# impromptuRong/hd_yolo

Measured on AMD Instinct MI355X. Metric: tiles/sec (640x640) fwd+bwd, higher is better.
Workload: dtype bf16; 1 GPU; metayolo yolov5s 8-class nuclei, 640x640 RGB tiles, batch 64/GPU, train step = fwd + DetLoss + bwd + all-reduce + SGD(nesterov); global_batch=64, parallelism=dp1, world_size=1, backend=none, hw_queues=4

## Files before the change

hd_yolo_amd/build.py:

```python
import os
import subprocess
import sys
from concurrent.futures import ThreadPoolExecutor

HERE = os.path.dirname(os.path.abspath(__file__))
CSRC = os.path.join(HERE, 'csrc')
OUT = os.path.join(CSRC, 'build')
LIB = os.path.join(OUT, 'libhdyolo_hip.so')
SOURCES = ['api.hip', 'conv_dispatch.hip', 'conv_igemm.hip', 'conv3x3.hip', 'conv3x3_c128.hip', 'conv3x3s2.hip', 'conv_deep.hip', 'conv_stem.hip', 'conv_wgrad.hip', 'conv_wgrad3x3.hip', 'conv_wgrad_deep.hip', 'conv_dgrad_s2.hip', 'conv1x1_bwd.hip', 'bn_act.hip', 'pool.hip', 'detect.hip', 'loss.hip', 'roi.hip', 'seg.hip', 'optim.hip', 'exec.hip']
FLAGS = ['--offload-arch=gfx950', '-O3', '-fPIC', '-std=c++17', '-ffp-contract=off', '-Wall', '-Wno-unused-function',
         '-I' + CSRC, '-I' + os.path.join(os.path.dirname(HERE), 'include')]


def _newer(a, bs):
    return os.path.exists(a) and all(os.path.getmtime(a) >= os.path.getmtime(b) for b in bs)


def build(force=False, verbose=True):
    os.makedirs(OUT, exist_ok=True)
    headers = [os.path.join(CSRC, h) for h in os.listdir(CSRC) if h.endswith('.h')]
    headers.append(os.path.join(os.path.dirname(HERE), 'include', 'hdyolo.h'))
    hipcc = os.environ.get('HIPCC', '/opt/rocm/bin/hipcc')

    def compile_one(src):
        s = os.path.join(CSRC, src)
        o = os.path.join(OUT, src.replace('.hip', '.o'))
        if not force and _newer(o, [s] + headers):
            return o
        cmd = [hipcc] + FLAGS + ['-c', s, '-o', o]
        if verbose:
            print(' '.join(cmd), flush=True)
        subprocess.check_call(cmd)
        return o

    with ThreadPoolExecutor(max_workers=min(6, os.cpu_count() or 1)) as ex:
        objs = list(ex.map(compile_one, SOURCES))
    if force or not _newer(LIB, objs):
        cmd = [hipcc, '--offload-arch=gfx950', '-shared', '-fPIC', '-o', LIB] + objs
        if verbose:
            print(' '.join(cmd), flush=True)
        subprocess.check_call(cmd)
    return LIB


if __name__ == '__main__':
    print(build(force='--force' in sys.argv))
```

hd_yolo_amd/csrc/api.hip:

```cpp
#include <stdarg.h>
#include <stdio.h>
#include <stdlib.h>
#include <string.h>

#include <atomic>

#include "common.h"
#include "hdyolo_internal.h"
#include "hdyolo.h"

int hdy_wgrad_reduce_launch(const float* partial, int splits, size_t slab_stride, int K, int Q, int mode, int C, int R, int S, float* grad,
                            int accumulate, hipStream_t st);
int hdy_pack_weight_launch(const hdy_pack_desc& d, hipStream_t st);
int hdy_pack_batch_launch(const hdy_pack_desc* table, int n, int total_blocks, hipStream_t st);

static thread_local char g_err[512] = "";

void hdy_set_error(const char* fmt, ...) {
    va_list ap;
    va_start(ap, fmt);
    vsnprintf(g_err, sizeof(g_err), fmt, ap);
    va_end(ap);
}

namespace {
struct OptDef { const char* name; int def; bool flag; };
const OptDef g_opt_def[HDY_OPT_COUNT] = {
    {"HDY_NO_CLASS_WALK", 0, true}, {"HDY_NO_CONV3X3", 0, true}, {"HDY_C3_GRID", 0, false}, {"HDY_NO_CONV3X3S2", 0, false},
    {"HDY_NO_DGRAD_S2", 0, false}, {"HDY_TILE_INTERLEAVE", 1, false}, {"HDY_NO_BIG_TILES", 0, true}, {"HDY_NO_STEM_KERNEL", 0, true},
    {"HDY_WGRAD_BLOCKS", 512, false}, {"HDY_NO_STEM_WGRAD", 0, true}, {"HDY_NO_WGRAD3X3", 0, true}, 
    {"HDY_LOSS_GRID", 2048, false}, {"HDY_NO_DEEP", 0, true}, {"HDY_NO_WGRAD_S2", 0, true}, {"HDY_NO_WGRAD_DEEP", 0, true}, {"HDY_DEEP_BN", 0, false}, {"HDY_DEEP_DEBUG", 0, false}, {"HDY_DEEP_ALL", 1, false}, {"HDY_DEEP_MIN_TILES", 160, false}, {"HDY_DEEP_WALK", 2, false}, {"HDY_NO_BN_REDUCE4", 0, true},
    {"HDY_WGRAD_TILE", 0, false}, {"HDY_SPPF_NO_KEYS", 0, true}, {"HDY_WGRAD_DEEP_KMIN", 192, false}, {"HDY_NO_CONV3X3_C128", 0, true}, {"HDY_NO_F1X1_96", 0, true},
};
std::atomic<int> g_opt[HDY_OPT_COUNT];
std::once_flag g_opt_once;
void opt_init() {
    std::call_once(g_opt_once, [] {
        for (int i = 0; i < HDY_OPT_COUNT; ++i) {
            const char* v = getenv(g_opt_def[i].name);
            g_opt[i].store(v ? (g_opt_def[i].flag ? 1 : atoi(v)) : g_opt_def[i].def, std::memory_order_relaxed);
        }
    });
}
int opt_index(const char* name) {
    for (int i = 0; name && i < HDY_OPT_COUNT; ++i)
        if (!strcmp(name, g_opt_def[i].name)) return i;
    return -1;
}
thread_local char g_disp_last[64] = "";
std::mutex g_disp_mu;
char g_disp_log[32768] = "";
size_t g_disp_len = 0;
thread_local char g_disp_copy[32768] = "";
}

int hdy_opt(int id) {
    opt_init();
    return g_opt[id].load(std::memory_order_relaxed);
}

void hdy_note_dispatch(const char* what) {
    snprintf(g_disp_last, sizeof(g_disp_last), "%s", what);
    const size_t n = strlen(g_disp_last);
    std::lock_guard<std::mutex> lock(g_disp_mu);
    if (g_disp_len + n + 2 < sizeof(g_disp_log)) {
        memcpy(g_disp_log + g_disp_len, g_disp_last, n);
        g_disp_log[g_disp_len + n] = ';';
        g_disp_log[g_disp_len + n + 1] = 0;
        g_disp_len += n + 1;
    }
}

namespace {

enum { KIND_FWD = 0, KIND_DGRAD = 1, KIND_STEM = 2 };

inline int velems(int dtype) { return dtype == HDY_BF16 ? 8 : 4; }
inline int bke(int dtype) { return 8 * velems(dtype); }
inline size_t esize(int dtype) { return dtype == HDY_BF16 ? 2 : 4; }

struct Axis { int taps, d0, rmax; };
inline Axis class_axis(int R, int pad, int a) {
    Axis ax = {0, 0, -1};
    for (int r = R - 1; r >= 0; --r)
        if (((a + pad - r) & 1) == 0) {
            if (ax.rmax < 0) { ax.rmax = r; ax.d0 = (a + pad - r) / 2; }
            ++ax.taps;
        }
    return ax;
}

inline bool dgrad_class_walk(int H, int W, int R, int S, int pad) {
    if (H % 2 || W % 2 || hdy_opt(HDY_OPT_NO_CLASS_WALK)) return false;
    for (int a = 0; a < 2; ++a)
        if (!class_axis(R, pad, a).taps || !class_axis(S, pad, a).taps) return false;
    return true;
}

inline size_t block_elems(int rows, int kd, int dtype) {
    const int bn = hdy_conv_bn_tile(rows);
    return (size_t)round_up(rows, bn) * round_up(kd, bke(dtype));
}

}

extern "C" {

const char* hdy_last_error(void) { return g_err; }

const char* hdy_last_dispatch(void) { return g_disp_last; }

const char* hdy_dispatch_log(void) {
    std::lock_guard<std::mutex> lock(g_disp_mu);
    memcpy(g_disp_copy, g_disp_log, g_disp_len + 1);
    return g_disp_copy;
}

void hdy_dispatch_log_reset(void) {
    std::lock_guard<std::mutex> lock(g_disp_mu);
    g_disp_log[0] = 0;
    g_disp_len = 0;
    g_disp_last[0] = 0;
}

int hdy_set_option(const char* name, int value) {
    const int i = opt_index(name);
    HDY_ARG(i >= 0, "set_option: unknown option %s", name ? name : "(null)");
    opt_init();
    return g_opt[i].exchange(value, std::memory_order_relaxed);
}

int hdy_get_option(const char* name) {
    const int i = opt_index(name);
    HDY_ARG(i >= 0, "get_option: unknown option %s", name ? name : "(null)");
    return hdy_opt(i);
}

int hdy_version(void) { return HDY_ABI_VERSION; }

int hdy_fastdiv_magic(unsigned d, unsigned* magic, int* shift) {
    HDY_ARG(d > 0 && magic && shift, "fastdiv_magic: d must be positive");
    hdy_magic(d, magic, shift);
    return HDY_OK;
}

int hdy_conv_out_dim(int in, int k, int stride, int pad) { return conv_out_dim(in, k, stride, pad); }

int hdy_conv_mtiles(long long M) { return (int)((M + 127) / 128); }

size_t hdy_conv_pack_elems(int K, int C, int R, int S, int stride, int pad, int kind, int dtype) {
    if (kind == KIND_FWD) return block_elems(K, R * S * C, dtype);
    if (kind == KIND_STEM) return block_elems(K, R * S * 4, dtype);
    if (stride == 1) return block_elems(C, R * S * K, dtype);
    size_t n = 0;
    for (int a = 0; a < 2; ++a)
        for (int b = 0; b < 2; ++b) {
            const Axis ah = class_axis(R, pad, a), aw = class_axis(S, pad, b);
            if (ah.taps && aw.taps) n += block_elems(C, ah.taps * aw.taps * K, dtype);
        }
    return n;
}

static hdy_pack_desc make_desc(const float* w_a, int K_a, const float* w_b, int K_b, void* out, int Kl, int C, int R, int S, int transpose,
                               int TH, int TW, int rbase, int rstep, int sbase, int sstep, int stem, int rows_total, int Kdp, int dtype,
                               int first_block) {
    hdy_pack_desc d = {};
    d.w_a = w_a; d.w_b = w_b; d.out = out; d.K_a = K_a; d.K_b = K_b; d.Kl = Kl; d.C = C; d.R = R; d.S = S; d.transpose = transpose;
    d.TH = TH; d.TW = TW; d.rbase = rbase; d.rstep = rstep; d.sbase = sbase; d.sstep = sstep; d.stem = stem; d.rows_total = rows_total;
    d.Kdp = Kdp; d.dtype = dtype; d.first_block = first_block;
    d.nblocks = cdiv((long long)rows_total * Kdp, 2048);
    return d;
}

int hdy_conv_pack_describe(const float* w_a, int K_a, const float* w_b, int K_b, int K, int C, int R, int S, int stride, int pad, int kind,
                           int dtype, void* out, hdy_pack_desc* descs, int first_block) {
    HDY_ARG(w_a && out && descs && K_a > 0 && K_b >= 0 && K >= K_a + K_b && C > 0 && R > 0 && S > 0, "conv_pack: bad args");
    HDY_ARG((K_b == 0) == (w_b == nullptr), "conv_pack: w_b / K_b mismatch");
    HDY_ARG(stride == 1 || stride == 2, "conv_pack: stride %d unsupported", stride);
    HDY_ARG(dtype == HDY_BF16 || dtype == HDY_F32, "conv_pack: unknown dtype %d", dtype);
    HDY_ARG(((long long)K + 256) * ((long long)R * S * ((long long)C + 256) + 64) < (1LL << 31), "conv_pack: weight too large for 32-bit packing indices");
    if (kind == KIND_FWD || kind == KIND_STEM) {
        const int stem = kind == KIND_STEM;
        HDY_ARG(!stem || (C == 3 && K_b == 0), "conv_pack: stem expects C == 3 and a single weight");
        const int kd = stem ? R * S * 4 : R * S * C;
        const int Kdp = round_up(kd, bke(dtype));
        const int rows_total = round_up(K, hdy_conv_bn_tile(K));
        descs[0] = make_desc(w_a, K_a, w_b, K_b, out, K, C, R, S, 0, R, stem ? 1 : S, 0, 1, 0, 1, stem, rows_total, Kdp, dtype, first_block);
        return 1;
    }
    HDY_ARG(kind == KIND_DGRAD, "conv_pack: unknown kind %d", kind);
    const int rows_total = round_up(C, hdy_conv_bn_tile(C));
    if (stride == 1) {
        const int Kdp = round_up(R * S * K, bke(dtype));
        descs[0] = make_desc(w_a, K_a, w_b, K_b, out, K, C, R, S, 1, R, S, R - 1, -1, S - 1, -1, 0, rows_total, Kdp, dtype, first_block);
        return 1;
    }
    size_t off = 0;
    int n = 0;
    for (int a = 0; a < 2; ++a)
        for (int b = 0; b < 2; ++b) {
            const Axis ah = class_axis(R, pad, a), aw = class_axis(S, pad, b);
            if (!ah.taps || !aw.taps) continue;
            const int Kdp = round_up(ah.taps * aw.taps * K, bke(dtype));
            descs[n] = make_desc(w_a, K_a, w_b, K_b, (char*)out + off * esize(dtype), K, C, R, S, 1, ah.taps, aw.taps, ah.rmax, -2, aw.rmax,
                                 -2, 0, rows_total, Kdp, dtype, first_block);
            first_block += descs[n].nblocks;
            off += (size_t)rows_total * Kdp;
            ++n;
        }
    return n;
}

int hdy_conv_pack(const float* w_a, int K_a, const float* w_b, int K_b, int K, int C, int R, int S, int stride, int pad, int kind,
                  int dtype, void* out, void* stream) {
    hdy_pack_desc d[4];
    const int n = hdy_conv_pack_describe(w_a, K_a, w_b, K_b, K, C, R, S, stride, pad, kind, dtype, out, d, 0);
    if (n < 0) return n;
    for (int i = 0; i < n; ++i) {
        const int rc = hdy_pack_weight_launch(d[i], (hipStream_t)stream);
        if (rc) return rc;
    }
    return HDY_OK;
}

int hdy_conv_pack_run(const hdy_pack_desc* descs_device, int ndesc, int total_blocks, void* stream) {
    HDY_ARG(descs_device && ndesc > 0 && total_blocks > 0, "conv_pack_run: bad args");
    return hdy_pack_batch_launch(descs_device, ndesc, total_blocks, (hipStream_t)stream);
}

int hdy_conv_fwd(const void* x, int ldx, const void* w_packed, const float* scale, const float* shift, const void* res, int ldr, void* y,
                 int ldy, float* stats, int stat_slabs, int N, int H, int W, int C, int K, int R, int S, int stride, int pad, int act, int accumulate,
                 int dtype, int out_f32, int stem, void* stream) {
    HDY_ARG(!stats || stat_slabs > 0, "conv_fwd: stats given with stat_slabs = %d", stat_slabs);
    HDY_ARG(stride >= 1 && R >= 1 && S >= 1 && pad >= 0, "conv_fwd: bad window");
    HDY_ARG(dtype == HDY_BF16 || dtype == HDY_F32, "conv_fwd: unknown dtype %d", dtype);
    ConvArgs a = {};
    a.x = x; a.w = w_packed; a.y = y; a.scale = scale; a.shift = shift; a.stats = stats; a.stat_cap = stat_slabs; a.res = res; a.ldr = ldr;
    HDY_ARG(!res || ldr >= K, "conv_fwd: residual pitch %d < K", ldr);
    a.N = N;
    a.Ho = hdy_conv_out_dim(H, R, stride, pad);
    a.Wo = hdy_conv_out_dim(W, S, stride, pad);
    HDY_ARG(a.Ho > 0 && a.Wo > 0, "conv_fwd: empty output");
    a.K = K; a.ldy = ldy;
    a.Hout = a.Ho; a.Wout = a.Wo; a.oh_mul = a.ow_mul = 1; a.oh_off = a.ow_off = 0; a.dense_out = 1;
    a.act = act; a.accumulate = accumulate;
    if (stem) {
        HDY_ARG(C == 3 && R == 6 && S == 6 && stride == 2 && pad == 2 && ldx == 4, "conv_fwd: stem expects C=3 k=6 s=2 p=2 on a 4-channel padded image");
        a.Hin = H + 2 * pad; a.Win = W + 2 * pad; a.C = 24; a.ldx = 4; a.span_pixels = 1;
        a.ih_mul = 2; a.iw_mul = 2; a.dh0 = 0; a.dw0 = 0; a.TH = 6; a.TW = 1;
        a.Kdp = round_up(6 * 24, bke(dtype));
        return hdy_conv_launch(a, dtype, out_f32, (hipStream_t)stream);
    }
    a.Hin = H; a.Win = W; a.C = C; a.ldx = ldx;
    a.ih_mul = stride; a.iw_mul = stride; a.dh0 = -pad; a.dw0 = -pad; a.TH = R; a.TW = S;
    a.Kdp = round_up(R * S * C, bke(dtype));
    return hdy_conv_launch(a, dtype, out_f32, (hipStream_t)stream);
}

static int dgrad_impl(const void* dy, int lddy, const void* w_packed_dgrad, void* dx, int lddx, int N, int H, int W, int C, int K, int R,
                      int S, int stride, int pad, int accumulate, int dtype, const hdy_stat_req* stats, int nstat, void* stream);

int hdy_conv_dgrad(const void* dy, int lddy, const void* w_packed_dgrad, void* dx, int lddx, int N, int H, int W, int C, int K, int R,
                   int S, int stride, int pad, int accumulate, int dtype, void* stream) {
    return dgrad_impl(dy, lddy, w_packed_dgrad, dx, lddx, N, H, W, C, K, R, S, stride, pad, accumulate, dtype, nullptr, 0, stream);
}

int hdy_conv_dgrad_stats(const void* dy, int lddy, const void* w_packed_dgrad, void* dx, int lddx, int N, int H, int W, int C, int K, int R,
                         int S, int stride, int pad, int accumulate, int dtype, const hdy_stat_req* stats, int nstat, void* stream) {
    HDY_ARG(nstat >= 0 && nstat <= 2 && (nstat == 0 || stats), "conv_dgrad_stats: bad request count");
    HDY_ARG(nstat == 0 || hdy_conv_dgrad_stat_slabs(N, H, W, C, K, R, S, stride, pad, dtype) > 0, "conv_dgrad_stats: this shape cannot serve statistics");
    return dgrad_impl(dy, lddy, w_packed_dgrad, dx, lddx, N, H, W, C, K, R, S, stride, pad, accumulate, dtype, stats, nstat, stream);
}

int hdy_conv_dgrad_stat_slabs(int N, int H, int W, int C, int K, int R, int S, int stride, int pad, int dtype) {
    if (dtype != HDY_BF16 || C % 8 || hdy_conv_bn_tile(C) > 64 || (stride != 1 && stride != 2)) return 0;
    if (stride == 2 && !dgrad_class_walk(H, W, R, S, pad)) return 0;
    ConvShape s = {};
    s.N = N; s.Ho = H / stride; s.Wo = W / stride; s.C = K; s.K = C; s.R = R; s.S = S; s.stride = 1; s.pad = -1; s.dtype = dtype;
    s.dense = stride == 1; s.ncls = stride == 2 ? 4 : 1;
    ConvPlan p;
    hdy_conv_igemm_plan(s, &p);
    return p.grid;
}

static int dgrad_impl(const void* dy, int lddy, const void* w_packed_dgrad, void* dx, int lddx, int N, int H, int W, int C, int K, int R,
                      int S, int stride, int pad, int accumulate, int dtype, const hdy_stat_req* stats, int nstat, void* stream) {
    HDY_ARG(stride == 1 || stride == 2, "conv_dgrad: stride %d unsupported", stride);
    HDY_ARG(dtype == HDY_BF16 || dtype == HDY_F32, "conv_dgrad: unknown dtype %d", dtype);
    const int Ho = hdy_conv_out_dim(H, R, stride, pad), Wo = hdy_conv_out_dim(W, S, stride, pad);
    HDY_ARG(Ho > 0 && Wo > 0, "conv_dgrad: empty dy");
    ConvArgs a = {};
    a.x = dy; a.y = dx; a.N = N; a.Hin = Ho; a.Win = Wo; a.C = K; a.ldx = lddy;
    a.K = C; a.ldy = lddx; a.Hout = H; a.Wout = W;
    a.ih_mul = a.iw_mul = 1; a.accumulate = accumulate;
    a.nstat = nstat;
    for (int r = 0; r < nstat; ++r)
        a.stat[r] = StatReq{stats[r].y, stats[r].ldy, stats[r].scale, stats[r].shift, stats[r].slabs, stats[r].c0, stats[r].c1, stats[r].act, stats[r].nslabs};
    if (stride == 1) {
        a.w = w_packed_dgrad;
        a.Ho = H; a.Wo = W; a.oh_mul = a.ow_mul = 1; a.dense_out = 1;
        a.dh0 = pad - (R - 1); a.dw0 = pad - (S - 1); a.TH = R; a.TW = S;
        a.Kdp = round_up(R * S * K, bke(dtype));
        return hdy_conv_launch(a, dtype, 0, (hipStream_t)stream);
    }
    const int rows_total = round_up(C, hdy_conv_bn_tile(C));
    size_t off = 0;
    if (dgrad_class_walk(H, W, R, S, pad)) {
        ConvArgs c = a;
        c.ncls = 4;
        c.Ho = H / 2; c.Wo = W / 2;
        c.oh_mul = c.ow_mul = 2; c.dense_out = 0;
        for (int ca = 0; ca < 2; ++ca)
            for (int cb = 0; cb < 2; ++cb) {
                const Axis ah = class_axis(R, pad, ca), aw = class_axis(S, pad, cb);
                const int i = ca * 2 + cb;
                const int Kdp = round_up(ah.taps * aw.taps * K, bke(dtype));
                c.c_dh[i] = ah.d0; c.c_dw[i] = aw.d0; c.c_TH[i] = ah.taps; c.c_TW[i] = aw.taps;
                c.c_nkb[i] = Kdp / bke(dtype); c.c_oh[i] = ca; c.c_ow[i] = cb; c.c_w[i] = (long long)off;
                off += (size_t)rows_total * Kdp;
            }
        c.w = w_packed_dgrad;
        c.dh0 = c.c_dh[0]; c.dw0 = c.c_dw[0]; c.TH = c.c_TH[0]; c.TW = c.c_TW[0]; c.oh_off = c.ow_off = 0;
        c.Kdp = c.c_nkb[0] * bke(dtype);
        int rc2 = HDY_OK;
        if (hdy_dgrad3x3s2_try(c, dtype, (hipStream_t)stream, &rc2)) return rc2;
        return hdy_conv_launch(c, dtype, 0, (hipStream_t)stream);
    }
    for (int ca = 0; ca < 2; ++ca)
        for (int cb = 0; cb < 2; ++cb) {
            const Axis ah = class_axis(R, pad, ca), aw = class_axis(S, pad, cb);
            ConvArgs c = a;
            c.Ho = (H - ca + 1) / 2; c.Wo = (W - cb + 1) / 2;
            c.oh_mul = c.ow_mul = 2; c.oh_off = ca; c.ow_off = cb; c.dense_out = 0;
            if (!ah.taps || !aw.taps) {
                HDY_ARG(false, "conv_dgrad: kernel %dx%d pad %d leaves a parity class without taps (unsupported)", R, S, pad);
            }
            if (c.Ho <= 0 || c.Wo <= 0) continue;
            c.dh0 = ah.d0; c.dw0 = aw.d0; c.TH = ah.taps; c.TW = aw.taps;
            c.Kdp = round_up(ah.taps * aw.taps * K, bke(dtype));
            c.w = (const char*)w_packed_dgrad + off * esize(dtype);
            off += (size_t)rows_total * c.Kdp;
            const int rc = hdy_conv_launch(c, dtype, 0, (hipStream_t)stream);
            if (rc) return rc;
        }
    return HDY_OK;
}

size_t hdy_conv_wgrad_workspace_bytes(int N, int H, int W, int C, int K, int R, int S, int stride, int pad, int dtype, int stem) {
    const int Ho = hdy_conv_out_dim(H, R, stride, pad), Wo = hdy_conv_out_dim(W, S, stride, pad);
    const int Q = stem ? R * S * 4 : R * S * C;
    int splits = 1, pps = 64;
    hdy_wgrad_plan(K, Q, (long long)N * Ho * Wo, dtype, &splits, &pps);
    if (stem) {
        const int g = hdy_wgrad_stem_grid(N, Ho, Wo, K, dtype);
        if (g > splits) splits = g;
    }
    size_t bytes = (size_t)splits * K * Q * sizeof(float);
    if (!stem && R == 3 && S == 3 && pad == 1) {
        const size_t b3 = hdy_wgrad3x3_workspace_bytes(N, Ho, Wo, C, K, stride, dtype);
        if (b3 > bytes) bytes = b3;
    }
    if (!stem) {
        const size_t bd = hdy_wgrad_deep_workspace_bytes(N, H, W, Ho, Wo, C, K, R, S, stride, dtype);
        if (bd > bytes) bytes = bd;
    }
    return bytes;
}

int hdy_conv_wgrad(const void* x, int ldx, const void* dy, int lddy, int N, int H, int W, int C, int K, int R, int S, int stride, int pad,
                   float* grad_a, int K_a, float* grad_b, int K_b, int accumulate, void* workspace, size_t ws_bytes, int dtype, int stem,
                   void* stream) {
    HDY_ARG(grad_a && K_a > 0 && K_a + K_b <= K && K_b >= 0 && (K_b == 0) == (grad_b == nullptr), "conv_wgrad: bad gradient split");
    HDY_ARG(dtype == HDY_BF16 || dtype == HDY_F32, "conv_wgrad: unknown dtype %d", dtype);
    HDY_ARG(workspace && ws_bytes >= hdy_conv_wgrad_workspace_bytes(N, H, W, C, K, R, S, stride, pad, dtype, stem), "conv_wgrad: workspace too small");
    WgradArgs a = {};
    a.x = x; a.dy = dy; a.partial = (float*)workspace;
    a.N = N; a.K = K; a.lddy = lddy;
    a.Ho = hdy_conv_out_dim(H, R, stride, pad);
    a.Wo = hdy_conv_out_dim(W, S, stride, pad);
    HDY_ARG(a.Ho > 0 && a.Wo > 0, "conv_wgrad: empty dy");
    if (stem) {
        HDY_ARG(C == 3 && R == 6 && S == 6 && stride == 2 && pad == 2 && ldx == 4, "conv_wgrad: stem expects C=3 k=6 s=2 p=2 on a 4-channel padded image");
        a.Hin = H + 2 * pad; a.Win = W + 2 * pad; a.C = 24; a.ldx = 4; a.span_pixels = 1;
        a.ih_mul = a.iw_mul = 2; a.dh0 = a.dw0 = 0; a.TH = 6; a.TW = 1;
    } else {
        a.Hin = H; a.Win = W; a.C = C; a.ldx = ldx;
        a.ih_mul = a.iw_mul = stride; a.dh0 = a.dw0 = -pad; a.TH = R; a.TW = S;
    }
    const int Q = a.TH * a.TW * a.C;
    const int stem_grid = stem ? hdy_wgrad_stem_grid(N, a.Ho, a.Wo, K, dtype) : 0;
    int rc;
    if (!stem && R == 3 && S == 3 && pad == 1 &&
        hdy_wgrad3x3_try(x, ldx, dy, lddy, N, H, W, a.Ho, a.Wo, C, K, stride, a.partial, dtype, (hipStream_t)stream, &a.splits, &rc)) {
    } else if (!stem && hdy_wgrad_deep_try(x, ldx, dy, lddy, N, H, W, a.Ho, a.Wo, C, K, R, S, stride, pad, a.partial, dtype, (hipStream_t)stream, &a.splits, &rc)) {
    } else if (stem_grid > 0) {
        a.splits = stem_grid;
        rc = hdy_wgrad_stem_launch(a, stem_grid, (hipStream_t)stream);
    } else {
        hdy_wgrad_plan(K, Q, (long long)N * a.Ho * a.Wo, dtype, &a.splits, &a.pix_per_split);
        rc = hdy_wgrad_launch(a, dtype, (hipStream_t)stream);
    }
    if (rc) return rc;
    const int mode = stem ? 1 : 0;
    rc = hdy_wgrad_reduce_launch(a.partial, a.splits, (size_t)K * Q, K_a, Q, mode, C, R, S, grad_a, accumulate, (hipStream_t)stream);
    if (rc) return rc;
    if (K_b) {
        rc = hdy_wgrad_reduce_launch(a.partial + (size_t)K_a * Q, a.splits, (size_t)K * Q, K_b, Q, mode, C, R, S, grad_b, accumulate,
                                     (hipStream_t)stream);
    }
    return rc;
}

int hdy_conv_wgrad_stem_fused_ok(int N, int H, int W, int K) {
    if (K != 16 && K != 32 && K != 64) return 0;
    const int Ho = hdy_conv_out_dim(H, 6, 2, 2), Wo = hdy_conv_out_dim(W, 6, 2, 2);
    return hdy_wgrad_stem_grid(N, Ho, Wo, K, HDY_BF16) > 0 ? 1 : 0;
}

int hdy_conv_wgrad_stem_fused(const void* x, const void* dz, int lddz, const void* y, int ldy, const float* scale, const float* shift, const float* mean,
                              const float* invstd, const float* c1, const float* c2, int N, int H, int W, int K, float* grad_a, int K_a, float* grad_b,
                              int K_b, int accumulate, void* workspace, size_t ws_bytes, void* stream) {
    HDY_ARG(x && dz && y && grad_a && K_a > 0 && K_a + K_b <= K && K_b >= 0 && (K_b == 0) == (grad_b == nullptr), "conv_wgrad_stem_fused: bad arguments");
    HDY_ARG(hdy_conv_wgrad_stem_fused_ok(N, H, W, K), "conv_wgrad_stem_fused: shape not served (K in {16, 32, 64}, output a multiple of 16 x 32)");
    HDY_ARG(workspace && ws_bytes >= hdy_conv_wgrad_workspace_bytes(N, H, W, 3, K, 6, 6, 2, 2, HDY_BF16, 1), "conv_wgrad_stem_fused: workspace too small");
    WgradArgs a = {};
    a.x = x; a.dy = dz; a.lddy = lddz; a.partial = (float*)workspace;
    a.y = y; a.ldy = ldy; a.bn_scale = scale; a.bn_shift = shift; a.bn_mean = mean; a.bn_invstd = invstd; a.bn_c1 = c1; a.bn_c2 = c2;
    a.N = N; a.K = K;
    a.Ho = hdy_conv_out_dim(H, 6, 2, 2);
    a.Wo = hdy_conv_out_dim(W, 6, 2, 2);
    a.Hin = H + 4; a.Win = W + 4; a.C = 24; a.ldx = 4; a.span_pixels = 1;
    a.ih_mul = a.iw_mul = 2; a.dh0 = a.dw0 = 0; a.TH = 6; a.TW = 1;
    const int Q = a.TH * a.TW * a.C;
    a.splits = hdy_wgrad_stem_grid(N, a.Ho, a.Wo, K, HDY_BF16);
    int rc = hdy_wgrad_stem_launch(a, a.splits, (hipStream_t)stream);
    if (rc) return rc;
    rc = hdy_wgrad_reduce_launch(a.partial, a.splits, (size_t)K * Q, K_a, Q, 1, 3, 6, 6, grad_a, accumulate, (hipStream_t)stream);
    if (rc) return rc;
    if (K_b) rc = hdy_wgrad_reduce_launch(a.partial + (size_t)K_a * Q, a.splits, (size_t)K * Q, K_b, Q, 1, 3, 6, 6, grad_b, accumulate, (hipStream_t)stream);
    return rc;
}

}
```

hd_yolo_amd/csrc/common.h:

```cpp
#pragma once
#include <hip/hip_runtime.h>
#include <stdint.h>
#include <stddef.h>

#include <mutex>

#define HDY_OK 0
#define HDY_EINVAL (-1)
#define HDY_EUNSUPPORTED (-2)

enum { HDY_F32 = 0, HDY_BF16 = 1 };

void hdy_set_error(const char* fmt, ...);

enum HdyOption {
    HDY_OPT_NO_CLASS_WALK,
    HDY_OPT_NO_CONV3X3,
    HDY_OPT_C3_GRID,
    HDY_OPT_NO_CONV3X3S2,
    HDY_OPT_NO_DGRAD_S2,
    HDY_OPT_TILE_INTERLEAVE,
    HDY_OPT_NO_BIG_TILES,
    HDY_OPT_NO_STEM_KERNEL,
    HDY_OPT_WGRAD_BLOCKS,
    HDY_OPT_NO_STEM_WGRAD,
    HDY_OPT_NO_WGRAD3X3,
    HDY_OPT_LOSS_GRID,
    HDY_OPT_NO_DEEP,
    HDY_OPT_NO_WGRAD_S2,
    HDY_OPT_NO_WGRAD_DEEP,
    HDY_OPT_DEEP_BN,
    HDY_OPT_DEEP_DEBUG,
    HDY_OPT_DEEP_ALL,
    HDY_OPT_DEEP_MIN_TILES,
    HDY_OPT_DEEP_WALK,
    HDY_OPT_NO_BN_REDUCE4,
    HDY_OPT_WGRAD_TILE,
    HDY_OPT_SPPF_NO_KEYS,
    HDY_OPT_WGRAD_DEEP_KMIN,
    HDY_OPT_NO_CONV3X3_C128,
    HDY_OPT_NO_F1X1_96,
    HDY_OPT_COUNT
};
int hdy_opt(int id);

void hdy_note_dispatch(const char* what);

#define HDY_ARG(cond, ...)                 \
    do {                                   \
        if (!(cond)) {                     \
            hdy_set_error(__VA_ARGS__);    \
            return HDY_EINVAL;             \
        }                                  \
    } while (0)

#define HDY_LAUNCH_CHECK(what)                                                       \
    do {                                                                             \
        hipError_t e__ = hipGetLastError();                                          \
        if (e__ != hipSuccess) {                                                     \
            hdy_set_error("%s: launch failed: %s", what, hipGetErrorString(e__));    \
            return (int)e__;                                                         \
        }                                                                            \
    } while (0)

typedef __bf16 bf16_t;
typedef int i32x4 __attribute__((ext_vector_type(4)));
typedef float f32x4 __attribute__((ext_vector_type(4)));
typedef __bf16 bf16x8 __attribute__((ext_vector_type(8)));
typedef __bf16 bf16x4 __attribute__((ext_vector_type(4)));

#if defined(__HIPCC__)
__device__ __forceinline__ float row_sum16(float v) {
#ifdef HDY_ROW_SUM_SHFL
    for (int m = 1; m < 16; m <<= 1) v += __shfl_xor(v, m);
    return v;
#endif
    v += __builtin_bit_cast(float, __builtin_amdgcn_update_dpp(0, __builtin_bit_cast(int, v), 0x128, 0xF, 0xF, true));
    v += __builtin_bit_cast(float, __builtin_amdgcn_update_dpp(0, __builtin_bit_cast(int, v), 0x124, 0xF, 0xF, true));
    v += __builtin_bit_cast(float, __builtin_amdgcn_update_dpp(0, __builtin_bit_cast(int, v), 0x122, 0xF, 0xF, true));
    v += __builtin_bit_cast(float, __builtin_amdgcn_update_dpp(0, __builtin_bit_cast(int, v), 0x121, 0xF, 0xF, true));
    return v;
}
#endif

struct PerDeviceOnce {
    std::once_flag flag[16];
    template <typename F> void run(F&& fn) {
        int dev = 0;
        (void)hipGetDevice(&dev);
        std::call_once(flag[dev & 15], fn);
    }
};

static inline int cdiv(long long a, long long b) { return (int)((a + b - 1) / b); }
static inline int round_up(int a, int b) { return (a + b - 1) / b * b; }

#ifdef __HIPCC__
union V16 {
    i32x4 i;
    f32x4 f;
    bf16x8 h;
};

__device__ __forceinline__ float silu_f(float u) { return u / (1.0f + __expf(-u)); }
__device__ __forceinline__ float sigmoid_f(float u) { return 1.0f / (1.0f + __expf(-u)); }

template <typename T> __device__ __forceinline__ float to_f32(T v);
template <> __device__ __forceinline__ float to_f32<float>(float v) { return v; }
template <> __device__ __forceinline__ float to_f32<bf16_t>(bf16_t v) { return (float)v; }
template <typename T> __device__ __forceinline__ T from_f32(float v);
template <> __device__ __forceinline__ float from_f32<float>(float v) { return v; }
template <> __device__ __forceinline__ bf16_t from_f32<bf16_t>(float v) { return (bf16_t)v; }

__device__ __forceinline__ int xcd_remap(int id, int n) {
    const int q = n >> 3, r = n & 7, x = id & 7, s = id >> 3;
    return (x < r ? x * (q + 1) : r * (q + 1) + (x - r) * q) + s;
}
__device__ __forceinline__ unsigned fdiv(unsigned n, unsigned mg, int sh) { return __umulhi(n << 1, mg) >> sh; }

__device__ __forceinline__ void glds16(const void* g, unsigned char* lds_wave_base) {
    __builtin_amdgcn_global_load_lds((const void __attribute__((address_space(1)))*)g,
                                     (void __attribute__((address_space(3)))*)lds_wave_base, 16, 0, 0);
}

__device__ __forceinline__ void lds_dma16(__amdgpu_buffer_rsrc_t r, unsigned voff, unsigned soff, unsigned char* lds_wave_base) {
    __builtin_amdgcn_raw_ptr_buffer_load_lds(r, (void __attribute__((address_space(3)))*)lds_wave_base, 16, (int)voff, (int)soff, 0, 0);
}

__device__ __forceinline__ void lds_dma16(__amdgpu_buffer_rsrc_t r, unsigned voff, unsigned soff, unsigned lds_byte) {
    __builtin_amdgcn_raw_ptr_buffer_load_lds(r, (void __attribute__((address_space(3)))*)(uintptr_t)lds_byte, 16, (int)voff, (int)soff, 0, 0);
}

__device__ __forceinline__ int fsw(int row) { return ((row >> 1) & 1) | (((row >> 3) & 1) << 1); }
__device__ __forceinline__ int fsw3(int row) { return (row & 6) ^ (((row >> 3) & 1) * 5); }

__device__ __forceinline__ float fast_sigmoid(float u) { return __builtin_amdgcn_rcpf(1.0f + __expf(-u)); }
__device__ __forceinline__ float dsilu_f(float u) {
    const float s = fast_sigmoid(u);
    return s * (1.0f + u * (1.0f - s));
}

template <typename T> __device__ __forceinline__ void unpack(const i32x4& v, float* f);
template <> __device__ __forceinline__ void unpack<float>(const i32x4& v, float* f) {
    V16 u; u.i = v;
#pragma unroll
    for (int i = 0; i < 4; ++i) f[i] = u.f[i];
}
template <> __device__ __forceinline__ void unpack<bf16_t>(const i32x4& v, float* f) {
    V16 u; u.i = v;
#pragma unroll
    for (int i = 0; i < 8; ++i) f[i] = (float)u.h[i];
}
template <typename T> __device__ __forceinline__ i32x4 pack(const float* f);
template <> __device__ __forceinline__ i32x4 pack<float>(const float* f) {
    V16 u;
#pragma unroll
    for (int i = 0; i < 4; ++i) u.f[i] = f[i];
    return u.i;
}
template <> __device__ __forceinline__ i32x4 pack<bf16_t>(const float* f) {
    V16 u;
#pragma unroll
    for (int i = 0; i < 8; ++i) u.h[i] = (bf16_t)f[i];
    return u.i;
}

#define VEC_OK(ptr, ld, VE) ((((uintptr_t)(ptr)) & 15) == 0 && (ld) % (VE) == 0)

#define S2_LDSR(dst, addr)                                                                             \
    do {                                                                                               \
        if constexpr (HAND) asm volatile("ds_read_b128 %0, %1" : "=v"(dst) : "v"(addr) : "memory");    \
        else dst = *(const i32x4*)(smem + ((addr) - lds0));                                            \
    } while (0)
#define S2_LGKM(n)                                                                                                       \
    do {                                                                                                                 \
        if constexpr (HAND) { asm volatile("s_waitcnt lgkmcnt(%0)" ::"n"(n) : "memory"); __builtin_amdgcn_sched_barrier(0); } \
    } while (0)
#define S2_BARRIER(lg)                                                                                                   \
    do {                                                                                                                 \
        if constexpr (HAND) { if (lg) asm volatile("s_waitcnt lgkmcnt(0)" ::: "memory"); __builtin_amdgcn_s_barrier(); asm volatile("" ::: "memory"); } \
        else __syncthreads();                                                                                            \
    } while (0)
#endif
```

hd_yolo_amd/csrc/hdyolo_internal.h:

```cpp
#pragma once
#include <type_traits>

#include "common.h"

struct StatReq {
    const void* y; int ldy;
    const float *scale, *shift;
    float* slabs;
    int c0, c1, act;
    int nslabs;
};

struct ConvArgs {
    const void* x;
    const void* w;
    void* y;
    const float* scale;
    const float* shift;
    float* stats;
    int stat_cap;
    const void* res;
    int ldr;
    int N, Hin, Win, C, ldx;
    int Ho, Wo, K, ldy;
    int Hout, Wout, oh_mul, oh_off, ow_mul, ow_off;
    int ih_mul, iw_mul, dh0, dw0, TH, TW;
    int Kd, Kdp, M;
    int act, accumulate, dense_out;
    int mtiles, ntiles, bn;
    int span_pixels;
    int pointwise;
    int vec_out;
    int nstat;
    StatReq stat[2];
    int ncls;
    int c_dh[4], c_dw[4], c_TH[4], c_TW[4], c_nkb[4], c_oh[4], c_ow[4];
    long long c_w[4];
    int uh0, uw0, UH, UW, utap;
    int tile_interleave;
    unsigned mg_howo, mg_wo, mg_c, mg_tw[4];
    int sh_howo, sh_wo, sh_c, sh_tw[4];
    int dbg;
};

struct ConvShape {
    int N, H, W;
    int Ho, Wo;
    int C, K, R, S, stride;
    int pad;
    int dense;
    int dtype;
    int stem;
    int stats;
    int ncls;
};
inline int hdy_conv_bn_tile(int K) { return K <= 32 ? 32 : (K <= 64 ? 64 : 128); }
inline int conv_out_dim(int in, int k, int stride, int pad) { return (in + 2 * pad - k) / stride + 1; }
inline ConvShape conv_shape(int N, int H, int W, int C, int K, int R, int S, int stride, int pad, int dtype, int stem, int stats) {
    return ConvShape{N, H, W, conv_out_dim(H, R, stride, pad), conv_out_dim(W, S, stride, pad), C, K, R, S, stride, pad, 1, dtype, stem, stats, 1};
}
inline long long conv_pixels(const ConvShape& s) { return (long long)s.N * s.Ho * s.Wo; }
inline int conv_taps(const ConvShape& s) { return s.stem ? 6 : s.R * s.S; }
inline bool conv_is(const ConvShape& s, int R, int stride, int pad) { return !s.stem && s.ncls <= 1 && s.R == R && s.S == R && s.stride == stride && s.pad == pad; }

enum ConvFamily { CONV_NONE = 0, CONV_STEM, CONV_3X3_C64, CONV_3X3_C128, CONV_3X3S2, CONV_DEEP, CONV_IGEMM };

struct ConvPlan {
    int family;
    int variant;
    int grid;
    int slabs;
    int bn;
    int interleave;
};

bool hdy_conv_stem_plan(const ConvShape& s, ConvPlan* p);
bool hdy_conv3x3_c64_plan(const ConvShape& s, ConvPlan* p);
bool hdy_conv3x3_c128_plan(const ConvShape& s, ConvPlan* p);
bool hdy_conv3x3s2_plan(const ConvShape& s, ConvPlan* p);
bool hdy_conv_deep_plan(const ConvShape& s, ConvPlan* p);
bool hdy_conv_igemm_plan(const ConvShape& s, ConvPlan* p);

enum { HDY_CONV_DECLINE = -100 };
int hdy_conv_stem_launch(const ConvArgs& a, const ConvPlan& p, int out_f32, hipStream_t st);
int hdy_conv3x3_c64_launch(const ConvArgs& a, const ConvPlan& p, int out_f32, hipStream_t st);
int hdy_conv3x3_c128_launch(const ConvArgs& a, const ConvPlan& p, int out_f32, hipStream_t st);
int hdy_conv3x3s2_launch(const ConvArgs& a, const ConvPlan& p, int out_f32, hipStream_t st);
int hdy_conv_deep_launch(const ConvArgs& a, const ConvPlan& p, int out_f32, hipStream_t st);
int hdy_conv_igemm_launch(const ConvArgs& a, const ConvPlan& p, int dtype, int out_f32, hipStream_t st);

inline int hdy_conv_take(const ConvArgs& a, const ConvPlan& p, bool fits, const char* who) {
    if (!fits && !a.stats) return HDY_CONV_DECLINE;
    HDY_ARG(fits, "%s: statistics requested, but this call does not fit the kernel their slabs were sized for (bf16 output, 16-byte aligned x/y/res rows; "
            "ldx=%d ldy=%d)", who, a.ldx, a.ldy);
    HDY_ARG(!a.stats || a.stat_cap == p.slabs, "%s: the statistics array holds %d slabs, this launch writes %d (a kernel-selection option changed between "
            "hdy_conv_stat_slabs and the launch?)", who, a.stat_cap, p.slabs);
    return HDY_OK;
}

inline bool rows_aligned(const ConvArgs& a, bool need_w) {
    return a.ldx % 8 == 0 && a.ldy % 8 == 0 && (((uintptr_t)a.x | (uintptr_t)a.y) & 15) == 0 && (!need_w || (((uintptr_t)a.w & 15) == 0 && a.Kdp % 8 == 0)) &&
           (!a.res || (a.ldr % 8 == 0 && ((uintptr_t)a.res & 15) == 0));
}

inline int epilogue_of(const ConvArgs& a) { return a.act == 1 ? 2 : ((a.scale || a.shift) ? 1 : 0); }

template <typename F> inline void with_stats_epi(bool stats, int epi, F&& f) {
    auto with_epi = [&](auto s) {
        if (epi == 2) f(s, std::integral_constant<int, 2>{});
        else if (epi == 1) f(s, std::integral_constant<int, 1>{});
        else f(s, std::integral_constant<int, 0>{});
    };
    if (stats) with_epi(std::true_type{});
    else with_epi(std::false_type{});
}

inline int hdy_launch_status(const char* who) {
    HDY_LAUNCH_CHECK(who);
    return HDY_OK;
}

inline void hdy_magic(unsigned d, unsigned* mg, int* sh) {
    int s = 0;
    while ((1ull << s) < d) ++s;
    *mg = (unsigned)((((unsigned long long)1 << (31 + s)) + d - 1) / d);
    *sh = s;
}

struct WgradArgs {
    const void* x;
    const void* dy;
    float* partial;
    int N, Hin, Win, C, ldx;
    int Ho, Wo, K, lddy;
    int ih_mul, iw_mul, dh0, dw0, TH, TW;
    int Q, P;
    int splits, pix_per_split;
    int ktiles, qtiles;
    int span_pixels;
    const void* y; int ldy;
    const float *bn_scale, *bn_shift, *bn_mean, *bn_invstd, *bn_c1, *bn_c2;
};

int hdy_wgrad_stem_grid(int N, int Ho, int Wo, int K, int dtype);
int hdy_wgrad_stem_launch(const WgradArgs& a, int grid, hipStream_t st);
int hdy_wgrad_launch(WgradArgs a, int dtype, hipStream_t st);
int hdy_wgrad_plan(int K, int Q, long long P, int dtype, int* splits, int* pix_per_split);
size_t hdy_wgrad3x3_workspace_bytes(int N, int Ho, int Wo, int C, int K, int stride, int dtype);
int hdy_wgrad3x3_try(const void* x, int ldx, const void* dy, int lddy, int N, int Hin, int Win, int Ho, int Wo, int C, int K, int stride, float* partial,
                     int dtype, hipStream_t st, int* splits, int* rc);
size_t hdy_wgrad_deep_workspace_bytes(int N, int Hin, int Win, int Ho, int Wo, int C, int K, int R, int S, int stride, int dtype);
int hdy_wgrad_deep_try(const void* x, int ldx, const void* dy, int lddy, int N, int Hin, int Win, int Ho, int Wo, int C, int K, int R, int S, int stride,
                       int pad, float* partial, int dtype, hipStream_t st, int* splits, int* rc);
int hdy_conv_launch(ConvArgs a, int dtype, int out_f32, hipStream_t st);
int hdy_dgrad3x3s2_try(const ConvArgs& a, int dtype, hipStream_t st, int* rc);
```

Before: 5429 tiles/s.

## Add wide-channel fused 4-class dgrad kernel for stride-2 3x3 convs

Adds a new persistent HIP kernel for the data gradient of stride-2 3x3 convs with C in {128,256,512} and K in {128,256}. It computes all four parity classes from one shared input patch in LDS, double-buffers the patch and weight slices with direct global-to-LDS loads, and issues MFMA bf16. The existing narrow dgrad path still gets first refusal, and any call it declines is routed here instead of the generic implicit-GEMM fallback. This is meant to cut redundant input loads and launch overhead on the wider backbone layers, at the cost of 1 block per CU occupancy, heavy LDS use and a fixed 256-block grid.

```diff
diff --git a/hd_yolo_amd/build.py b/hd_yolo_amd/build.py
--- a/hd_yolo_amd/build.py
+++ b/hd_yolo_amd/build.py
@@ -7,7 +7,7 @@
 CSRC = os.path.join(HERE, 'csrc')
 OUT = os.path.join(CSRC, 'build')
 LIB = os.path.join(OUT, 'libhdyolo_hip.so')
-SOURCES = ['api.hip', 'conv_dispatch.hip', 'conv_igemm.hip', 'conv3x3.hip', 'conv3x3_c128.hip', 'conv3x3s2.hip', 'conv_deep.hip', 'conv_stem.hip', 'conv_wgrad.hip', 'conv_wgrad3x3.hip', 'conv_wgrad_deep.hip', 'conv_dgrad_s2.hip', 'conv1x1_bwd.hip', 'bn_act.hip', 'pool.hip', 'detect.hip', 'loss.hip', 'roi.hip', 'seg.hip', 'optim.hip', 'exec.hip']
+SOURCES = ['api.hip', 'conv_dispatch.hip', 'conv_igemm.hip', 'conv3x3.hip', 'conv3x3_c128.hip', 'conv3x3s2.hip', 'conv_deep.hip', 'conv_stem.hip', 'conv_wgrad.hip', 'conv_wgrad3x3.hip', 'conv_wgrad_deep.hip', 'conv_dgrad_s2.hip', 'conv_dgrad_s2_wide.hip', 'conv1x1_bwd.hip', 'bn_act.hip', 'pool.hip', 'detect.hip', 'loss.hip', 'roi.hip', 'seg.hip', 'optim.hip', 'exec.hip']
 FLAGS = ['--offload-arch=gfx950', '-O3', '-fPIC', '-std=c++17', '-ffp-contract=off', '-Wall', '-Wno-unused-function',
          '-I' + CSRC, '-I' + os.path.join(os.path.dirname(HERE), 'include')]
 
diff --git a/hd_yolo_amd/csrc/api.hip b/hd_yolo_amd/csrc/api.hip
--- a/hd_yolo_amd/csrc/api.hip
+++ b/hd_yolo_amd/csrc/api.hip
@@ -31,6 +31,7 @@
     {"HDY_WGRAD_BLOCKS", 512, false}, {"HDY_NO_STEM_WGRAD", 0, true}, {"HDY_NO_WGRAD3X3", 0, true}, 
     {"HDY_LOSS_GRID", 2048, false}, {"HDY_NO_DEEP", 0, true}, {"HDY_NO_WGRAD_S2", 0, true}, {"HDY_NO_WGRAD_DEEP", 0, true}, {"HDY_DEEP_BN", 0, false}, {"HDY_DEEP_DEBUG", 0, false}, {"HDY_DEEP_ALL", 1, false}, {"HDY_DEEP_MIN_TILES", 160, false}, {"HDY_DEEP_WALK", 2, false}, {"HDY_NO_BN_REDUCE4", 0, true},
     {"HDY_WGRAD_TILE", 0, false}, {"HDY_SPPF_NO_KEYS", 0, true}, {"HDY_WGRAD_DEEP_KMIN", 192, false}, {"HDY_NO_CONV3X3_C128", 0, true}, {"HDY_NO_F1X1_96", 0, true},
+    {"HDY_NO_DGRAD_S2_WIDE", 0, true}, {"HDY_DGRAD_S2_WIDE_MIN_ITEMS", 256, false},
 };
 std::atomic<int> g_opt[HDY_OPT_COUNT];
 std::once_flag g_opt_once;
@@ -324,6 +325,7 @@
         c.Kdp = c.c_nkb[0] * bke(dtype);
         int rc2 = HDY_OK;
         if (hdy_dgrad3x3s2_try(c, dtype, (hipStream_t)stream, &rc2)) return rc2;
+        if (hdy_dgrad3x3s2_wide_try(c, dtype, (hipStream_t)stream, &rc2)) return rc2;
         return hdy_conv_launch(c, dtype, 0, (hipStream_t)stream);
     }
     for (int ca = 0; ca < 2; ++ca)
diff --git a/hd_yolo_amd/csrc/common.h b/hd_yolo_amd/csrc/common.h
--- a/hd_yolo_amd/csrc/common.h
+++ b/hd_yolo_amd/csrc/common.h
@@ -40,6 +40,8 @@
     HDY_OPT_WGRAD_DEEP_KMIN,
     HDY_OPT_NO_CONV3X3_C128,
     HDY_OPT_NO_F1X1_96,
+    HDY_OPT_NO_DGRAD_S2_WIDE,
+    HDY_OPT_DGRAD_S2_WIDE_MIN_ITEMS,
     HDY_OPT_COUNT
 };
 int hdy_opt(int id);
diff --git a/hd_yolo_amd/csrc/conv_dgrad_s2_wide.hip b/hd_yolo_amd/csrc/conv_dgrad_s2_wide.hip
--- /dev/null
+++ b/hd_yolo_amd/csrc/conv_dgrad_s2_wide.hip
@@ -0,0 +1,310 @@
+#include <stdlib.h>
+
+#include "common.h"
+#include "hdyolo_internal.h"
+
+__device__ uint4 g_hdy_zero16_d2w[4];
+__device__ uint4 g_hdy_dump_d2w[512];
+
+namespace {
+
+#ifndef DW_ABL
+#define DW_ABL 0
+#endif
+constexpr int NTHR = 512;
+constexpr int MAXPIX = 304;
+constexpr int PATCH_B = MAXPIX * 64;
+constexpr int SLICE_B = 64 * 64;
+constexpr int STAGE_B = PATCH_B + 9 * SLICE_B;
+constexpr int STG_B = 256 * 128;
+constexpr int SMEM_B = 2 * STAGE_B + STG_B;
+
+struct WideGeo {
+    int TW, TH, PW, PPIX, npos;
+    int tiles_w, tiles_h, ncb, items;
+    int inv_tw, inv_pw;
+    int nstage;
+};
+
+#define DW_LDSR(dst, addr, imm) asm volatile("ds_read_b128 %0, %1 offset:%2" : "=v"(dst) : "v"(addr), "n"(imm) : "memory")
+#define DW_LGKM0()                                                  \
+    do {                                                            \
+        asm volatile("s_waitcnt lgkmcnt(0)" ::: "memory");          \
+        __builtin_amdgcn_sched_barrier(0);                          \
+    } while (0)
+#define DW_BARRIER()                                                \
+    do {                                                            \
+        asm volatile("s_waitcnt lgkmcnt(0)" ::: "memory");          \
+        __builtin_amdgcn_s_barrier();                               \
+        asm volatile("" ::: "memory");                              \
+        __builtin_amdgcn_sched_barrier(0);                          \
+    } while (0)
+
+__device__ __forceinline__ int swz64(int row, int chunk) { return chunk ^ (((row >> 2) & 1) << 1); }
+
+__global__ __launch_bounds__(NTHR, 1) void dgrad3x3s2_wide_kernel(const ConvArgs p, const WideGeo g) {
+    extern __shared__ __attribute__((aligned(16))) unsigned char smem[];
+    const unsigned lds0 = (unsigned)(uintptr_t)(const __attribute__((address_space(3))) unsigned char*)smem;
+    const int tid = threadIdx.x, lane = tid & 63, wave = tid >> 6;
+    const int fr = lane & 15, fq = lane >> 4;
+    const int cgp = wave & 1, fgrp = wave >> 1;
+    const int wg = xcd_remap(blockIdx.x, gridDim.x);
+    if (wg >= g.items) return;
+
+    const bf16_t* __restrict__ x = (const bf16_t*)p.x;
+    const bf16_t* __restrict__ w = (const bf16_t*)p.w;
+    const unsigned char* zero = (const unsigned char*)g_hdy_zero16_d2w;
+    const int per_img = g.tiles_w * g.tiles_h;
+    constexpr unsigned CLS_OF = 0u | 1u << 2 | 1u << 4 | 2u << 6 | 2u << 8 | 3u << 10 | 3u << 12 | 3u << 14 | 3u << 16;
+    constexpr unsigned TAP_OF = 0u | 0u << 2 | 1u << 4 | 0u << 6 | 1u << 8 | 0u << 10 | 1u << 12 | 2u << 14 | 3u << 16;
+
+    auto item_geo = [&](int t, int& n, int& i0, int& j0, int& cb) {
+        cb = t % g.ncb;
+        const int tile = t / g.ncb;
+        n = tile / per_img;
+        const int rem = tile - n * per_img;
+        const int th = rem / g.tiles_w;
+        i0 = th * g.TH;
+        j0 = (rem - th * g.tiles_w) * g.TW;
+    };
+
+    auto issue_stage = [&](int t, int ks, int buf) {
+        int tv = tid;
+        asm volatile("" : "+v"(tv));
+        const int wv = __builtin_amdgcn_readfirstlane(tv >> 6);
+        int n, i0, j0, cb;
+        item_geo(t, n, i0, j0, cb);
+        unsigned char* dst = smem + buf * STAGE_B;
+        const bf16_t* org = x + (((long long)n * p.Hin + i0) * p.Win + j0) * p.ldx + ks * 32;
+        const int nslot = g.PPIX * 4;
+#pragma unroll
+        for (int i = 0; i < 3; ++i) {
+            if (wv * 64 + NTHR * i >= nslot) break;
+            const int s = tv + NTHR * i;
+            const int pix = s >> 2;
+            const int py = (pix * g.inv_pw) >> 16, px = pix - py * g.PW;
+            const bool ok = pix < g.PPIX && i0 + py < p.Hin && j0 + px < p.Win;
+            const void* src = ok ? (const void*)(org + ((long long)py * p.Win + px) * p.ldx + swz64(pix, s & 3) * 8) : (const void*)zero;
+            glds16(src, dst + (wv * 64 + NTHR * i) * 16);
+        }
+#pragma unroll
+        for (int i = 0; i < 5; ++i) {
+            const int sl = (wv >> 2) + 2 * i;
+            if (sl >= 9) break;
+            const int cls = (CLS_OF >> (2 * sl)) & 3, tap = (TAP_OF >> (2 * sl)) & 3;
+            const int s = tv & 255;
+            const int c = s >> 2;
+            const bf16_t* src = w + p.c_w[cls] + (long long)(cb * 64 + c) * (p.c_nkb[cls] * 64) + tap * p.C + ks * 32 + swz64(c, s & 3) * 8;
+            glds16(src, dst + PATCH_B + sl * SLICE_B + (wv & 3) * 1024);
+        }
+    };
+
+    unsigned dyo[4][4];
+#pragma unroll
+    for (int f = 0; f < 4; ++f) {
+        int pos = (fgrp * 4 + f) * 16 + fr;
+        pos = pos < g.npos ? pos : g.npos - 1;
+        const int row = (pos * g.inv_tw) >> 16, col = pos - row * g.TW;
+#pragma unroll
+        for (int sh = 0; sh < 4; ++sh) {
+            const int pix = (row + (sh >> 1)) * g.PW + col + (sh & 1);
+            dyo[f][sh] = pix * 64 + (swz64(pix, fq) << 4);
+        }
+    }
+    const unsigned wlane = PATCH_B + cgp * 2048 + fr * 64 + (swz64(fr, fq) << 4);
+
+    f32x4 acc[4][4][2];
+
+    auto compute = [&](int buf) {
+        const unsigned pb = lds0 + buf * STAGE_B;
+        const unsigned wb_ = pb + wlane;
+        V16 d0[4], d1[4], wa[2][2], wb[2][2];
+#define RD_DY(d, sh)                                                            \
+        _Pragma("unroll") for (int f = 0; f < 4; ++f) DW_LDSR(d[f].i, pb + dyo[f][sh], 0)
+#define RD_W(dst, sl)                                                           \
+        do {                                                                    \
+            DW_LDSR(dst[0].i, wb_, (sl) * SLICE_B);                             \
+            DW_LDSR(dst[1].i, wb_, (sl) * SLICE_B + 1024);                      \
+        } while (0)
+#define MF(d, wv, cls)                                                          \
+        _Pragma("unroll") for (int f = 0; f < 4; ++f) {                         \
+            acc[cls][f][0] = __builtin_amdgcn_mfma_f32_16x16x32_bf16(wv[0].h, d[f].h, acc[cls][f][0], 0, 0, 0);   \
+            acc[cls][f][1] = __builtin_amdgcn_mfma_f32_16x16x32_bf16(wv[1].h, d[f].h, acc[cls][f][1], 0, 0, 0);   \
+        }
+        if (DW_ABL & 4) return;
+        RD_DY(d0, 0); RD_W(wa[0], 0); RD_W(wa[1], 1);
+        DW_LGKM0();
+        RD_W(wb[0], 3); RD_W(wb[1], 5);
+        MF(d0, wa[0], 0) MF(d0, wa[1], 1)
+        DW_LGKM0();
+        RD_DY(d1, 1); RD_W(wa[0], 2); RD_W(wa[1], 6);
+        MF(d0, wb[0], 2) MF(d0, wb[1], 3)
+        DW_LGKM0();
+        RD_DY(d0, 2); RD_W(wb[0], 4); RD_W(wb[1], 7);
+        MF(d1, wa[0], 1) MF(d1, wa[1], 3)
+        DW_LGKM0();
+        RD_DY(d1, 3); RD_W(wa[0], 8);
+        MF(d0, wb[0], 2) MF(d0, wb[1], 3)
+        DW_LGKM0();
+        MF(d1, wa[0], 3)
+#undef RD_DY
+#undef RD_W
+#undef MF
+    };
+
+    const int st_ch = tid & 7, st_pos = tid >> 3;
+    int prc[4];
+#pragma unroll
+    for (int j = 0; j < 4; ++j) {
+        const int pos = st_pos + 64 * j;
+        const int row = (pos * g.inv_tw) >> 16, col = pos - row * g.TW;
+        prc[j] = pos < g.npos ? (row << 8 | col) : -1;
+    }
+    bf16_t* const dump = (bf16_t*)g_hdy_dump_d2w + tid * 8;
+    bf16_t* yp0[4];
+    bool ok[4];
+    long long ystep_h = 0, ystep_w = 0;
+    V16 u[4];
+
+    auto out_ptrs = [&](int t) {
+        int n, i0, j0, cb;
+        item_geo(t, n, i0, j0, cb);
+        bf16_t* base = (bf16_t*)p.y + (((long long)n * p.Hout + 2 * i0) * p.Wout + 2 * j0) * p.ldy + cb * 64 + st_ch * 8;
+        ystep_w = p.ldy;
+        ystep_h = (long long)p.Wout * p.ldy;
+#pragma unroll
+        for (int j = 0; j < 4; ++j) {
+            const int row = prc[j] >> 8, col = prc[j] & 255;
+            ok[j] = prc[j] >= 0 && i0 + row < p.Ho && j0 + col < p.Wo;
+            yp0[j] = base + ((long long)(2 * row) * p.Wout + 2 * col) * p.ldy;
+        }
+    };
+    auto cls_ptr = [&](int j, int cls) { return ok[j] ? yp0[j] + (cls >> 1) * ystep_h + (cls & 1) * ystep_w : dump; };
+    auto load_old = [&](int cls) {
+#pragma unroll
+        for (int j = 0; j < 4; ++j) asm volatile("global_load_dwordx4 %0, %1, off" : "=v"(u[j].i) : "v"(cls_ptr(j, cls)) : "memory");
+    };
+
+    auto epilogue = [&]() {
+        const unsigned sS = lds0 + 2 * STAGE_B;
+#pragma unroll
+        for (int cls = 0; cls < 4; ++cls) {
+#pragma unroll
+            for (int f = 0; f < 4; ++f)
+#pragma unroll
+                for (int gg = 0; gg < 2; ++gg) {
+                    const int pos = (fgrp * 4 + f) * 16 + fr;
+                    const int slot = (cgp * 8 + gg * 4 + fq) ^ fr;
+                    const f32x4 a = acc[cls][f][gg];
+                    const bf16x4 o = {(bf16_t)a[0], (bf16_t)a[1], (bf16_t)a[2], (bf16_t)a[3]};
+                    const long long o8 = __builtin_bit_cast(long long, o);
+                    asm volatile("ds_write_b64 %0, %1" ::"v"(sS + pos * 128 + slot * 8), "v"(o8) : "memory");
+                }
+            DW_BARRIER();
+            V16 v[4];
+#pragma unroll
+            for (int j = 0; j < 4; ++j) {
+                const int pos = st_pos + 64 * j;
+                DW_LDSR(v[j].i, sS + pos * 128 + ((st_ch ^ ((pos & 15) >> 1)) << 4), 0);
+            }
+            DW_LGKM0();
+#pragma unroll
+            for (int j = 0; j < 4; ++j)
+                if ((st_pos + 64 * j) & 1) v[j].i = i32x4{v[j].i[2], v[j].i[3], v[j].i[0], v[j].i[1]};
+            if (p.accumulate) {
+                if (cls == 0) asm volatile("s_waitcnt vmcnt(0)" ::: "memory");
+                else asm volatile("s_waitcnt vmcnt(4)" ::: "memory");
+                __builtin_amdgcn_sched_barrier(0);
+#pragma unroll
+                for (int j = 0; j < 4; ++j)
+#pragma unroll
+                    for (int e = 0; e < 8; ++e) v[j].h[e] = (bf16_t)((float)v[j].h[e] + (float)u[j].h[e]);
+                if (cls < 3) load_old(cls + 1);
+            }
+#pragma unroll
+            for (int j = 0; j < 4; ++j)
+                if (!(DW_ABL & 8)) *(i32x4*)cls_ptr(j, cls) = v[j].i;
+            DW_BARRIER();
+        }
+    };
+
+    issue_stage(wg, 0, 0);
+    int cur = 0;
+    for (int t = wg; t < g.items; t += (int)gridDim.x) {
+#pragma unroll
+        for (int c = 0; c < 4; ++c)
+#pragma unroll
+            for (int f = 0; f < 4; ++f) acc[c][f][0] = acc[c][f][1] = f32x4{0.f, 0.f, 0.f, 0.f};
+        for (int ks = 0; ks < g.nstage; ++ks, cur ^= 1) {
+            if (ks == 0 && t != wg) asm volatile("s_waitcnt vmcnt(16)" ::: "memory");
+            else asm volatile("s_waitcnt vmcnt(0)" ::: "memory");
+            DW_BARRIER();
+            if (DW_ABL & 1) {
+            } else if (ks + 1 < g.nstage) issue_stage(t, ks + 1, cur ^ 1);
+            else if (t + (int)gridDim.x < g.items) issue_stage(t + (int)gridDim.x, 0, cur ^ 1);
+            if (ks == g.nstage - 1) {
+                out_ptrs(t);
+                if (p.accumulate) load_old(0);
+            }
+            compute(cur);
+        }
+        if (!(DW_ABL & 16)) epilogue();
+    }
+}
+
+void wide_tile(int Ho, int Wo, int* tw_out, int* th_out) {
+    int best = 1 << 30, btw = 1, bth = 1;
+    for (int tw = 1; tw <= Wo && tw <= 64; ++tw) {
+        int th = 256 / tw;
+        if (th > Ho) th = Ho;
+        while (th > 1 && (th + 1) * (tw + 1) > MAXPIX) --th;
+        if ((th + 1) * (tw + 1) > MAXPIX) continue;
+        const int n = cdiv(Wo, tw) * cdiv(Ho, th);
+        if (n <= best) { best = n; btw = tw; bth = th; }
+    }
+    *tw_out = btw;
+    *th_out = bth;
+}
+
+}
+
+int hdy_dgrad3x3s2_wide_try(const ConvArgs& a, int dtype, hipStream_t st, int* rc) {
+    if (hdy_opt(HDY_OPT_NO_DGRAD_S2) == 1 || hdy_opt(HDY_OPT_NO_DGRAD_S2_WIDE)) return 0;
+    if (dtype != HDY_BF16 || a.ncls != 4 || a.nstat != 0 || a.res || a.scale || a.shift || a.act != 0 || a.stats) return 0;
+    if (!(a.C == 128 || a.C == 256 || a.C == 512) || !(a.K == 128 || a.K == 256)) return 0;
+    if (a.Hin != a.Ho || a.Win != a.Wo || a.Hout != 2 * a.Ho || a.Wout != 2 * a.Wo) return 0;
+    const int np = a.C / 64;
+    static const int nth[4] = {1, 1, 2, 2}, ntw[4] = {1, 2, 1, 2}, oh[4] = {0, 0, 1, 1}, ow[4] = {0, 1, 0, 1};
+    for (int c = 0; c < 4; ++c)
+        if (a.c_dh[c] != 0 || a.c_dw[c] != 0 || a.c_TH[c] != nth[c] || a.c_TW[c] != ntw[c] || a.c_oh[c] != oh[c] || a.c_ow[c] != ow[c] ||
+            a.c_nkb[c] != nth[c] * ntw[c] * np || a.c_w[c] % 8)
+            return 0;
+    if (a.ldx % 8 || a.ldy % 8 || ((uintptr_t)a.x & 15) || ((uintptr_t)a.y & 15) || ((uintptr_t)a.w & 15)) return 0;
+    WideGeo g;
+    wide_tile(a.Ho, a.Wo, &g.TW, &g.TH);
+    g.PW = g.TW + 1;
+    g.PPIX = (g.TH + 1) * g.PW;
+    g.npos = g.TW * g.TH;
+    g.tiles_w = cdiv(a.Wo, g.TW);
+    g.tiles_h = cdiv(a.Ho, g.TH);
+    g.ncb = a.K / 64;
+    const long long items = (long long)a.N * g.tiles_w * g.tiles_h * g.ncb;
+    if (items < hdy_opt(HDY_OPT_DGRAD_S2_WIDE_MIN_ITEMS) || items >= (1LL << 30)) return 0;
+    g.items = (int)items;
+    g.inv_tw = 65536 / g.TW + 1;
+    g.inv_pw = 65536 / g.PW + 1;
+    g.nstage = a.C / 32;
+    hdy_note_dispatch("dgrad3x3s2_wide");
+    static PerDeviceOnce attr_once;
+    attr_once.run([&] { (void)hipFuncSetAttribute((const void*)dgrad3x3s2_wide_kernel, hipFuncAttributeMaxDynamicSharedMemorySize, SMEM_B); });
+    const int grid = g.items < 256 ? g.items : 256;
+    hipLaunchKernelGGL(dgrad3x3s2_wide_kernel, dim3(grid), dim3(NTHR), SMEM_B, st, a, g);
+    const int e = (int)hipGetLastError();
+    if (e != (int)hipSuccess) {
+        hdy_set_error("dgrad3x3s2_wide: launch failed: %s", hipGetErrorString((hipError_t)e));
+        *rc = e;
+        return 1;
+    }
+    *rc = HDY_OK;
+    return 1;
+}
diff --git a/hd_yolo_amd/csrc/hdyolo_internal.h b/hd_yolo_amd/csrc/hdyolo_internal.h
--- a/hd_yolo_amd/csrc/hdyolo_internal.h
+++ b/hd_yolo_amd/csrc/hdyolo_internal.h
@@ -154,3 +154,4 @@
                        int pad, float* partial, int dtype, hipStream_t st, int* splits, int* rc);
 int hdy_conv_launch(ConvArgs a, int dtype, int out_f32, hipStream_t st);
 int hdy_dgrad3x3s2_try(const ConvArgs& a, int dtype, hipStream_t st, int* rc);
+int hdy_dgrad3x3s2_wide_try(const ConvArgs& a, int dtype, hipStream_t st, int* rc);
```

After: 5430 tiles/s (median of 3 runs). Within noise of the previous version (+0.0%).
